# CEA-LIST/runia_core

Measured on AMD Instinct MI355X. Metric: OOD scores/sec, LaREM 16-MC PCA-256 (ResNet-18 layer4 latent 512x4x4), higher is better.
Workload: dtype f64

## Files before the change

### include/runia_hip.h

```cpp
#ifndef RUNIA_HIP_H
#define RUNIA_HIP_H

#include <stddef.h>
#include <stdint.h>

#ifdef __cplusplus
extern "C" {
#endif

#define RUNIA_OK 0
#define RUNIA_E_INVALID (-1)
#define RUNIA_E_LAUNCH (-2)
#define RUNIA_E_NODEVICE (-3)
#define RUNIA_E_WORKSPACE (-4)

typedef void* runia_stream_t;

int runia_abi_version(void);
const char* runia_error_string(int code);
int runia_device_count(void);
int runia_clock_probe(uint64_t* out4, int chain, runia_stream_t stream);
int runia_time_next_launch(void* start_event, void* stop_event);

int runia_mc_stack_f32(const float* x, const float* rand, int64_t rand_image_stride, float* out,
// ... 81 lines not shown
size_t runia_knn_prepared_workspace_bytes(int64_t N, int64_t M, int64_t D, int k);
int runia_knn_kth_prepared_f32(const float* q, const float* bank, const void* state, size_t state_bytes, float* score,
                               void* workspace, size_t workspace_bytes, int64_t N, int64_t M, int64_t D, int k,
                               runia_stream_t stream);
int runia_knn_kth_f32(const float* q, const float* bank, float* score, void* workspace,
                      size_t workspace_bytes, int64_t N, int64_t M, int64_t D, int k,
                      runia_stream_t stream);

int runia_kde_score_f64(const double* train, const double* x, double* score, int64_t M, int64_t N,
                        int64_t D, double bandwidth, runia_stream_t stream);
int runia_kde_score_kernel_f64(const double* train, const double* x, double* score, int64_t M, int64_t N, int64_t D,
                               double bandwidth, int kind, runia_stream_t stream);
int runia_row_sqnorm_f64(const double* x, double* out, int64_t N, int64_t D, runia_stream_t stream);
size_t runia_kde_workspace_bytes(int64_t N, int64_t M);
int runia_kde_score_packed_f64(const double* packed_train_t, const double* train_sqnorm, const double* x,
                               double* score, void* workspace, size_t workspace_bytes, int64_t M, int64_t N,
                               int64_t D, double bandwidth, runia_stream_t stream);

int runia_mc_entropy_supported(int H, int W, int n_mc, int k);
size_t runia_mc_entropy_workspace_bytes(int64_t N, int H, int W, int n_mc);
int runia_mc_mask_table_f32(const float* rand, int64_t rand_image_stride, void* workspace,
                            size_t workspace_bytes, int64_t N, int H, int W, int n_mc, double drop_prob,
                            int block_size, runia_stream_t stream);
int runia_mc_stack_table_f32(const float* x, const float* rand, int64_t rand_image_stride, float* z,
                             void* workspace, size_t workspace_bytes, int64_t N, int C, int H, int W, int n_mc,
                             double drop_prob, int block_size, runia_stream_t stream);
int runia_mc_entropy_from_table_f32(const float* x, const void* workspace, size_t workspace_bytes, double* h,
                                    float* z_out, double* zero_fill, int64_t N, int C, int H, int W, int n_mc,
                                    int k, double min_dist, runia_stream_t stream);
int runia_mc_entropy_f32(const float* x, const float* rand, int64_t rand_image_stride, double* h,
                         float* z_out, double* zero_fill, void* workspace, size_t workspace_bytes, int64_t N,
                         int C, int H, int W, int n_mc, double drop_prob, int block_size, int k, double min_dist,
                         runia_stream_t stream);
int runia_mc_draws_f32(float* out, int64_t N, int n_mc, int H, int W, uint64_t seed, int64_t first_image,
                       runia_stream_t stream);
int runia_mc_mask_table_counter_f32(uint64_t seed, int64_t first_image, void* workspace, size_t workspace_bytes,
                                    int64_t N, int H, int W, int n_mc, double drop_prob, int block_size,
                                    int redraw_dead_layers, runia_stream_t stream);
int runia_mc_entropy_counter_f32(const float* x, uint64_t seed, int64_t first_image, double* h, float* z_out,
                                 double* zero_fill, void* workspace, size_t workspace_bytes, int64_t N, int C, int H,
                                 int W, int n_mc, double drop_prob, int block_size, int k, double min_dist,
                                 int redraw_dead_layers, runia_stream_t stream);
int runia_pca_md_score_f64(const double* h, const double* packed_ct, const double* bias,
                           const double* scale, const double* md_mean, const double* packed_p,
                           double* score, double* y_out, int64_t N, int64_t D, int64_t n,
                           runia_stream_t stream);
size_t runia_proj_sq_workspace_bytes(int64_t N);
int runia_proj_sq_accumulate_f64(const double* h, const double* packed_m, const double* c, double* score,
                                 int64_t N, int64_t D, int64_t r, runia_stream_t stream);
int runia_proj_sq_score_f64(const double* h, const double* packed_m, const double* c, double* score,
                            void* workspace, size_t workspace_bytes, int64_t N, int64_t D, int64_t r,
                            runia_stream_t stream);

size_t runia_covariance_workspace_bytes(int64_t N, int64_t D);
int runia_covariance_f64(const double* x, double* mean, double* cov, void* workspace,
                         size_t workspace_bytes, int64_t N, int64_t D, runia_stream_t stream);
int runia_covariance_f32in(const float* x, double* mean, double* cov, void* workspace,
                           size_t workspace_bytes, int64_t N, int64_t D, runia_stream_t stream);

int runia_roi_align_f32(const float* input, const float* boxes, const int* batch_idx, float* out, int64_t K, int64_t B,
                        int C, int H, int W, int PH, int PW, double spatial_scale, int sampling_ratio, int aligned,
                        runia_stream_t stream);
int runia_nchw_to_nhwc_f32(const float* in, float* out, int64_t B, int C, int64_t HW, runia_stream_t stream);
int runia_roi_mc_entropy_supported(int PH, int PW, int n_mc, int k, int sampling_ratio);
size_t runia_roi_mc_entropy_workspace_bytes(int64_t K, int PH, int PW, int n_mc, int sampling_ratio);
int runia_roi_mc_entropy_f32(const float* feat_nhwc, const float* boxes, const int* batch_idx, const float* rand,
// ... 176 lines not shown
```

### runia_core_amd/_hip.py

```python
from __future__ import annotations

import contextlib
import ctypes
import os
import threading
from ctypes import c_char_p, c_double, c_float, c_int, c_int64, c_size_t, c_uint64, c_void_p
from typing import NamedTuple, Optional, Union

import numpy as np
import torch

from . import config as _config

_LIB_PATH = os.path.join(os.path.dirname(os.path.abspath(__file__)), "librunia_hip.so")
_lib: Optional[ctypes.CDLL] = None

_SIGNATURES = {
    "runia_abi_version": (c_int, []),
    "runia_error_string": (c_char_p, [c_int]),
    "runia_device_count": (c_int, []),
    "runia_clock_probe": (c_int, [c_void_p, c_int, c_void_p]),
    "runia_time_next_launch": (c_int, [c_void_p, c_void_p]),
    "runia_mc_stack_f32": (
        c_int,
# ... 56 lines not shown
    "runia_knn_kth_prepared_f32": (c_int, [c_void_p, c_void_p, c_void_p, c_size_t, c_void_p, c_void_p, c_size_t, c_int64, c_int64,
                                           c_int64, c_int, c_void_p]),
    "runia_knn_kth_f32": (
        c_int,
        [c_void_p, c_void_p, c_void_p, c_void_p, c_size_t, c_int64, c_int64, c_int64, c_int, c_void_p],
    ),
    "runia_kde_score_f64": (c_int, [c_void_p, c_void_p, c_void_p, c_int64, c_int64, c_int64, c_double, c_void_p]),
    "runia_row_sqnorm_f64": (c_int, [c_void_p, c_void_p, c_int64, c_int64, c_void_p]),
    "runia_kde_workspace_bytes": (c_size_t, [c_int64, c_int64]),
    "runia_kde_score_packed_f64": (
        c_int,
        [c_void_p, c_void_p, c_void_p, c_void_p, c_void_p, c_size_t, c_int64, c_int64, c_int64, c_double, c_void_p],
    ),
    "runia_mc_entropy_supported": (c_int, [c_int, c_int, c_int, c_int]),
    "runia_mc_entropy_workspace_bytes": (c_size_t, [c_int64, c_int, c_int, c_int]),
    "runia_mc_mask_table_f32": (
        c_int,
        [c_void_p, c_int64, c_void_p, c_size_t, c_int64, c_int, c_int, c_int, c_double, c_int, c_void_p],
    ),
    "runia_mc_stack_table_f32": (
        c_int,
        [c_void_p, c_void_p, c_int64, c_void_p, c_void_p, c_size_t, c_int64, c_int, c_int, c_int, c_int, c_double, c_int,
         c_void_p],
    ),
    "runia_mc_entropy_from_table_f32": (
        c_int,
        [c_void_p, c_void_p, c_size_t, c_void_p, c_void_p, c_void_p, c_int64, c_int, c_int, c_int, c_int, c_int,
         c_double, c_void_p],
    ),
    "runia_mc_entropy_f32": (
        c_int,
        [c_void_p, c_void_p, c_int64, c_void_p, c_void_p, c_void_p, c_void_p, c_size_t, c_int64, c_int, c_int, c_int,
         c_int, c_double, c_int, c_int, c_double, c_void_p],
    ),
    "runia_mc_draws_f32": (c_int, [c_void_p, c_int64, c_int, c_int, c_int, c_uint64, c_int64, c_void_p]),
    "runia_mc_mask_table_counter_f32": (
        c_int,
        [c_uint64, c_int64, c_void_p, c_size_t, c_int64, c_int, c_int, c_int, c_double, c_int, c_int, c_void_p],
    ),
    "runia_mc_entropy_counter_f32": (
        c_int,
        [c_void_p, c_uint64, c_int64, c_void_p, c_void_p, c_void_p, c_void_p, c_size_t, c_int64, c_int, c_int, c_int,
         c_int, c_double, c_int, c_int, c_double, c_int, c_void_p],
    ),
    "runia_select_hist_f32": (c_int, [c_void_p, c_void_p, c_int64, ctypes.c_uint32, ctypes.c_uint32, c_int, c_void_p]),
    "runia_cholesky_f32": (c_int, [c_void_p, c_void_p, c_int64, c_int64, c_double, c_void_p]),
    "runia_cholesky_f64": (c_int, [c_void_p, c_void_p, c_int64, c_int64, c_double, c_void_p]),
    "runia_gmm_log_prob_workspace_bytes": (c_size_t, [c_int64, c_int64, c_int]),
    "runia_gmm_log_prob_f32": (c_int, [c_void_p, c_void_p, c_void_p, c_void_p, c_void_p, c_void_p, c_void_p, c_size_t, c_int64,
                                       c_int64, c_int, c_void_p]),
    "runia_ood_metrics_workspace_bytes": (c_size_t, [c_int64]),
    "runia_ood_metrics_f64": (c_int, [c_void_p, c_int64, c_void_p, c_int64, c_void_p, c_void_p, c_size_t, c_void_p]),
    "runia_ood_metrics_f32": (c_int, [c_void_p, c_int64, c_void_p, c_int64, c_void_p, c_void_p, c_size_t, c_void_p]),
    "runia_ood_clf_curve_f64": (
        c_int, [c_void_p, c_int64, c_void_p, c_int64, c_void_p, c_void_p, c_void_p, c_void_p, c_void_p, c_size_t, c_void_p]),
    "runia_ood_clf_curve_f32": (
        c_int, [c_void_p, c_int64, c_void_p, c_int64, c_void_p, c_void_p, c_void_p, c_void_p, c_void_p, c_size_t, c_void_p]),
    "runia_eigh_workspace_bytes": (c_size_t, [c_int64]),
    "runia_eigh_init_f64": (c_int, [c_void_p, c_void_p, c_int64, c_void_p, c_size_t, c_void_p]),
    "runia_eigh_sweep_f64": (c_int, [c_void_p, c_void_p, c_int64, c_void_p, c_size_t, c_void_p, c_void_p]),
    "runia_eigh_block_padded": (c_int64, [c_int64]),
    "runia_eigh_block_workspace_bytes": (c_size_t, [c_int64]),
    "runia_eigh_block_init_f64": (c_int, [c_void_p, c_void_p, c_int64, c_void_p, c_size_t, c_void_p]),
    "runia_eigh_block_sweep_f64": (c_int, [c_void_p, c_void_p, c_int64, c_void_p, c_size_t, c_void_p, c_void_p]),
    "runia_matmul_f64": (c_int, [c_void_p, c_void_p, c_void_p, c_int64, c_int64, c_int64, c_int, c_void_p]),
    "runia_p2p_buffer_bytes": (c_size_t, [c_int, c_size_t]),
# ... 803 lines not shown
               min_dist: float = 1e-5, want_samples: bool = False, out: Optional[torch.Tensor] = None,
               kernel_events: Optional[list] = None, zero_fill: Optional[torch.Tensor] = None,
               table: Optional[torch.Tensor] = None):
    lib = load_library()
    require_gpu()
    assert x.is_cuda and x.dtype == torch.float32 and x.dim() == 4
    x = x.contiguous()
    n, c, hh, ww = x.shape
    if table is not None:
        h = torch.empty((n, c), dtype=torch.float64, device=x.device) if out is None else out
        assert h.is_cuda and h.dtype == torch.float64 and h.shape == (n, c) and h.is_contiguous()
        z = torch.empty((n * n_mc, c), dtype=torch.float32, device=x.device) if want_samples else None
        ws_bytes = int(lib.runia_mc_entropy_workspace_bytes(n, hh, ww, n_mc))
        assert table.is_cuda and table.numel() >= ws_bytes and n <= 65535
        if zero_fill is not None:
            assert zero_fill.is_cuda and zero_fill.dtype == torch.float64 and zero_fill.shape == (n,) and zero_fill.is_contiguous()
        args = (x.data_ptr(), table.data_ptr(), ws_bytes, h.data_ptr(), _ptr(z), _ptr(zero_fill), n, c, hh, ww, n_mc, int(k),
                float(min_dist))
        if kernel_events is not None:
            kernel_events.append(_timed_call("runia_mc_entropy_from_table_f32", *args))
        else:
            launch("runia_mc_entropy_from_table_f32", *args)
        return (h, z) if want_samples else h
    counter = rand if isinstance(rand, CounterDraws) else None
    rand, stride = _draws(None if counter is not None else rand, n, n_mc, hh, ww)
    if out is None:
        h = torch.empty((n, c), dtype=torch.float64, device=x.device)
    else:
        assert out.is_cuda and out.dtype == torch.float64 and out.shape == (n, c) and out.is_contiguous()
        h = out
    z = torch.empty((n * n_mc, c), dtype=torch.float32, device=x.device) if want_samples else None
    if zero_fill is not None:
        assert zero_fill.is_cuda and zero_fill.dtype == torch.float64 and zero_fill.shape == (n,) and zero_fill.is_contiguous()
    ws_bytes = int(lib.runia_mc_entropy_workspace_bytes(min(65535, n), hh, ww, n_mc))
    ws = torch.empty(max(ws_bytes, 16), dtype=torch.uint8, device=x.device)
    if counter is not None:
        seed, redraw = int(counter.seed) & (2**64 - 1), int(bool(counter.redraw_dead_layers))
    for done, m in _image_slices(n):
        xp, hp = x.data_ptr() + done * c * hh * ww * 4, h.data_ptr() + done * c * 8
        rp = None if rand is None else rand.data_ptr() + done * stride * 4
        zp = None if z is None else z.data_ptr() + done * n_mc * c * 4
        zf = None if zero_fill is None else zero_fill.data_ptr() + done * 8
        if kernel_events is not None:
            if counter is not None:
                launch("runia_mc_mask_table_counter_f32", seed, int(counter.first_image) + done, ws.data_ptr(), ws_bytes, m, hh,
                       ww, n_mc, float(drop_prob), int(block_size), redraw)
            else:
                launch("runia_mc_mask_table_f32", rp, stride, ws.data_ptr(), ws_bytes, m, hh, ww, n_mc, float(drop_prob),
                       int(block_size))
            kernel_events.append(_timed_call("runia_mc_entropy_from_table_f32", xp, ws.data_ptr(), ws_bytes, hp, zp, zf, m, c, hh,
                                             ww, n_mc, int(k), float(min_dist)))
        elif counter is not None:
            launch("runia_mc_entropy_counter_f32", xp, seed, int(counter.first_image) + done, hp, zp, zf, ws.data_ptr(), ws_bytes,
                   m, c, hh, ww, n_mc, float(drop_prob), int(block_size), int(k), float(min_dist), redraw)
        else:
            launch("runia_mc_entropy_f32", xp, rp, stride, hp, zp, zf, ws.data_ptr(), ws_bytes, m, c, hh, ww, n_mc,
                   float(drop_prob), int(block_size), int(k), float(min_dist))
    return (h, z) if want_samples else h


@_device_guard()
def proj_sq_accumulate(h: torch.Tensor, packed_m: torch.Tensor, c: torch.Tensor, r: int, out: torch.Tensor) -> torch.Tensor:
    require_gpu()
    assert h.is_cuda and h.dtype == torch.float64 and h.dim() == 2
    h = h.contiguous()
    nrow, d = h.shape
    assert out.is_cuda and out.dtype == torch.float64 and out.shape == (nrow,) and out.is_contiguous()
    launch("runia_proj_sq_accumulate_f64", h.data_ptr(), packed_m.data_ptr(), c.data_ptr(), out.data_ptr(), nrow, d, int(r))
    return out


@_device_guard()
def pca_md_score(h: torch.Tensor, packed_ct: Optional[torch.Tensor], bias: Optional[torch.Tensor],
                 scale: Optional[torch.Tensor], md_mean: torch.Tensor, packed_p: torch.Tensor, n: int,
                 want_projection: bool = False, out: Optional[torch.Tensor] = None):
    require_gpu()
    assert h.is_cuda and h.dtype == torch.float64 and h.dim() == 2
    h = h.contiguous()
    nrow, d = h.shape
    if out is None:
        s = torch.empty((nrow,), dtype=torch.float64, device=h.device)
    else:
        assert out.is_cuda and out.dtype == torch.float64 and out.shape == (nrow,) and out.is_contiguous()
        s = out
    y = torch.empty((nrow, n), dtype=torch.float64, device=h.device) if want_projection else None
    launch("runia_pca_md_score_f64", h.data_ptr(), _ptr(packed_ct), _ptr(bias), _ptr(scale), md_mean.data_ptr(),
           packed_p.data_ptr(), s.data_ptr(), _ptr(y), nrow, d, n)
    return (s, y) if want_projection else s


# ... 635 lines not shown
```

### runia_core_amd/csrc/fused.hip

```cpp
#include "common.hpp"
#include "entropy_core.hpp"
#include "mfma_f64_tile.hpp"
#include "philox.hpp"
#include "div_consts.hpp"

namespace {

using namespace runia_entropy;
using namespace runia_mfma;

constexpr int kMaxMC = 64;
typedef float f2 __attribute__((ext_vector_type(2)));

__device__ __forceinline__ void layer_consts(int cnt, int& m, float& flag, float& zh, float& zl) {
  const int a = cnt ? __ffs(cnt) - 1 : 0;
  m = cnt >> a;
  flag = __uint_as_float((unsigned)(127 - a) << 23);
  zh = cnt ? __uint_as_float(runia_div::kDivHi[(m - 1) >> 1]) : NAN;
  zl = cnt ? __uint_as_float(runia_div::kDivLo[(m - 1) >> 1]) : 0.f;
}

__device__ __forceinline__ float add_f32(float a, float b) {
  float r;
  asm("v_add_f32 %0, %1, %2" : "=v"(r) : "v"(a), "v"(b));
// ... 7 lines not shown
}

template <int HT, int WT>
__host__ __device__ constexpr int mask_slot(int p) {
  if constexpr (HT % 2 == 0) {
    const int y = p / WT, xw = p - y * WT;
    return ((y >> 1) * WT + xw) * 2 + (y & 1);
  } else {
    return p;
  }
}

template <int HT, int WT>
__host__ __device__ constexpr int slot_position(int slot) {
  if constexpr (HT % 2 == 0) {
    const int e = slot & 1, t = slot >> 1;
    const int k = t / WT, xw = t - k * WT;
    return (2 * k + e) * WT + xw;
  } else {
    return slot;
  }
}

template <int HT, int WT>
__device__ __forceinline__ unsigned long long columns_below(int k) {
  unsigned long long row = (k >= 64) ? ~0ull : ((1ull << k) - 1ull), m = 0ull;
#pragma unroll
  for (int y = 0; y < HT; ++y) m |= row << (y * WT);
  return m;
}

constexpr int kMaskBitsWaves = 4;

template <int HT, int WT, int NP, bool REDRAW = false>
__global__ __launch_bounds__(64 * kMaskBitsWaves) void mc_mask_bits_kernel(const float* __restrict__ rnd,
                                                                           int64_t rand_stride,
                                                                           float* __restrict__ table, int64_t N,
                                                                           int n_mc, float gamma, int block_size,
                                                                           int identity, int sort_layers,
                                                                           uint64_t rng_seed, int64_t first_image) {
  constexpr int HW = HT * WT;
  static_assert(HW <= 64 && NP <= 64, "one drop layer per 64-bit word");
  constexpr bool DIV = (64 % HW == 0);
  constexpr int WORDS = (NP * HW + 63) / 64;
  constexpr unsigned long long FULL = (HW == 64) ? ~0ull : ((1ull << HW) - 1ull);
  const int lane = threadIdx.x & 63;
  const int64_t img = (int64_t)blockIdx.x * kMaskBitsWaves + (threadIdx.x >> 6);
  if (img >= N) return;
  const int bit0 = lane * HW, word0 = bit0 >> 6, off = bit0 & 63;
  const int pad = block_size / 2;

  auto seeds_of = [&](unsigned attempt) -> unsigned long long {
    float d[WORDS];
    if (rnd) {
      const float* r = rnd + img * rand_stride;
#pragma unroll
      for (int t = 0; t < WORDS; ++t) {
        const int i = lane + 64 * t;
        d[t] = (i < n_mc * HW) ? r[i] : 1.0f;
      }
    } else {
#pragma unroll
      for (int q = 0; q < (WORDS + 3) / 4; ++q) {
        const runia_philox::u4 b = runia_philox::lane_block(rng_seed, (uint64_t)(first_image + img), lane, q, attempt);
#pragma unroll
        for (int j = 0; j < 4; ++j) {
          const int t = 4 * q + j;
          if (t < WORDS) d[t] = (lane + 64 * t < n_mc * HW) ? runia_philox::component(b, j) : 1.0f;
        }
      }
    }
    unsigned long long lo = 0ull, hi = 0ull;
#pragma unroll
    for (int t = 0; t < WORDS; ++t) {
      const unsigned long long w = __ballot(d[t] < gamma);
      if (t == word0) lo = w;
      if (!DIV && t == word0 + 1) hi = w;
    }
    unsigned long long sd = lo >> off;
    if (!DIV && off + HW > 64) sd |= hi << (64 - off);
    return sd & FULL;
// ... 6 lines not shown
      hx |= (ox >= 0) ? ((seed >> ox) & columns_below<HT, WT>(WT - ox))
                      : ((seed << -ox) & ~columns_below<HT, WT>(-ox) & FULL);
    }
    unsigned long long dropped = 0ull;
    for (int dy = 0; dy < block_size; ++dy) {
      const int oy = dy - pad;
      if (oy >= HT || -oy >= HT) continue;
      dropped |= (oy >= 0) ? (hx >> (oy * WT)) : ((hx << (-oy * WT)) & FULL);
    }
    return ~dropped & FULL;
  };

  unsigned long long keep = identity ? FULL : keep_of(seeds_of(0u));
  if (REDRAW && !identity && !rnd) {
    for (unsigned attempt = 1; attempt <= 16u; ++attempt) {
      if (__ballot(lane < n_mc && keep == 0ull) == 0ull) break;
      const unsigned long long again = keep_of(seeds_of(attempt));
      if (keep == 0ull) keep = again;
    }
  }
  const int cnt = __popcll(keep);
  int m;
  float flag, zh, zl;
  layer_consts(cnt, m, flag, zh, zl);
  const int key = m ? m : 127;
  int rank = 0;
#pragma unroll
  for (int j = 0; j < NP; ++j) {
    const int o = __shfl(key, j, 64);
    rank += (j < n_mc) && ((o < key) || (o == key && j < lane));
  }
  if (!sort_layers) rank = lane;
  if (lane >= n_mc) return;
  float* out = table + img * (int64_t)(n_mc * (HW + 2));
  float* rec = out + rank * HW;
  if constexpr (HW % 4 == 0) {
#pragma unroll
    for (int c = 0; c < HW / 4; ++c) {
      float4 v;
      v.x = ((keep >> slot_position<HT, WT>(4 * c)) & 1ull) ? flag : 0.f;
      v.y = ((keep >> slot_position<HT, WT>(4 * c + 1)) & 1ull) ? flag : 0.f;
      v.z = ((keep >> slot_position<HT, WT>(4 * c + 2)) & 1ull) ? flag : 0.f;
      v.w = ((keep >> slot_position<HT, WT>(4 * c + 3)) & 1ull) ? flag : 0.f;
      reinterpret_cast<float4*>(rec)[c] = v;
    }
  } else {
#pragma unroll
    for (int q = 0; q < HW; ++q) rec[q] = ((keep >> slot_position<HT, WT>(q)) & 1ull) ? flag : 0.f;
  }
  out[n_mc * HW + rank] = zh;
  out[n_mc * (HW + 1) + rank] = zl;
}

#ifndef K1_BLOCK
#define K1_BLOCK 128
#endif
constexpr int kK1Block = K1_BLOCK;

struct RoiSource {
  const float* nhwc;
  const unsigned* table;
  int64_t image_bytes;
  int C;
  int roi_dwords;
};

template <int HT, int WT, int G>
__device__ __forceinline__ void roi_load_map(float (&u)[HT * WT], const RoiSource* __restrict__ src, int64_t roi, int c) {
  typedef const __attribute__((address_space(4))) unsigned* cptr;
  cptr tab = (cptr)(src->table + roi * (int64_t)src->roi_dwords);
  const unsigned image = tab[0];
  const __amdgpu_buffer_rsrc_t rsrc = __builtin_amdgcn_make_buffer_rsrc(
      const_cast<float*>(src->nhwc) + (int64_t)image * (src->image_bytes / 4), 0, (int)src->image_bytes, 0x00020000);
  const int voff = c * 4;
  cptr rows = tab + 8, cols = tab + 8 + 4 * (HT * G);
  constexpr float count = (float)(G * G);
  constexpr int SX = WT * G, SY = HT * G;
  unsigned ox_lo[SX], ox_hi[SX];
  float hx[SX], lx[SX];
#pragma unroll
  for (int sx = 0; sx < SX; ++sx) {
    ox_lo[sx] = cols[4 * sx];
    ox_hi[sx] = cols[4 * sx + 1];
    hx[sx] = __uint_as_float(cols[4 * sx + 2]);
// ... 14 lines not shown
        for (int sx = 0; sx < SX; ++sx) { tl[sx][0] = th[sx][0]; tl[sx][1] = th[sx][1]; }
      } else {
#pragma unroll
        for (int sx = 0; sx < SX; ++sx) {
          tl[sx][0] = __builtin_bit_cast(float, __builtin_amdgcn_raw_buffer_load_b32(rsrc, voff, (int)(oy_lo + ox_lo[sx]), 0));
          tl[sx][1] = __builtin_bit_cast(float, __builtin_amdgcn_raw_buffer_load_b32(rsrc, voff, (int)(oy_lo + ox_hi[sx]), 0));
        }
      }
#pragma unroll
      for (int sx = 0; sx < SX; ++sx) {
        th[sx][0] = __builtin_bit_cast(float, __builtin_amdgcn_raw_buffer_load_b32(rsrc, voff, (int)(oy_hi + ox_lo[sx]), 0));
        th[sx][1] = __builtin_bit_cast(float, __builtin_amdgcn_raw_buffer_load_b32(rsrc, voff, (int)(oy_hi + ox_hi[sx]), 0));
      }
      cur_lo = oy_lo;
      cur_hi = oy_hi;
    }
    __builtin_amdgcn_sched_barrier(0);
#pragma unroll
    for (int sx = 0; sx < SX; ++sx) {
      const float w1 = hy * hx[sx], w2 = hy * lx[sx], w3 = ly * hx[sx], w4 = ly * lx[sx];
      const float val = w1 * tl[sx][0] + w2 * tl[sx][1] + w3 * th[sx][0] + w4 * th[sx][1];
      float& bin = acc[(sy / G) * WT + (sx / G)];
      bin += val;
      asm volatile("" : "+v"(bin));
    }
  }
#pragma unroll
  for (int p = 0; p < HT * WT; ++p) u[p] = acc[p] / count;
}

#ifndef K1_IMGS
#define K1_IMGS 1
#endif
template <int HT, int WT, int NP, int K, bool FULL, bool ENTROPY, int ROI_G>
__device__ __forceinline__ void mc_entropy_item(const float* __restrict__ x, const float* __restrict__ table,
                                                double* __restrict__ h, float* __restrict__ z_out,
                                                double* __restrict__ zero_fill, int64_t N, int C, int n_mc_rt,
                                                double min_dist, double const_term, double inv_n, int64_t img, int c) {
  constexpr int HW = HT * WT;
  constexpr bool PAIRS = (HT % 2 == 0);
  const int n_mc = FULL ? NP : n_mc_rt;
  if (img >= N) return;
  if (zero_fill && c == 0) zero_fill[img] = 0.0;
  if (c >= C) return;
  const float* mk = table + img * (int64_t)(n_mc * (HW + 2));
  const float* zhs = mk + n_mc * HW;
  const float* zls = zhs + n_mc;
  float u[HW];
  if constexpr (ROI_G > 0) {
    roi_load_map<HT, WT, ROI_G>(u, reinterpret_cast<const RoiSource*>(x), img, c);
  } else {
    const float* xc = x + (img * C + c) * (int64_t)HW;
    if constexpr (HW % 4 == 0) {
#pragma unroll
      for (int p = 0; p < HW / 4; ++p) {
        const float4 v = reinterpret_cast<const float4*>(xc)[p];
        u[4 * p] = v.x; u[4 * p + 1] = v.y; u[4 * p + 2] = v.z; u[4 * p + 3] = v.w;
      }
    } else {
#pragma unroll
      for (int p = 0; p < HW; ++p) u[p] = xc[p];
    }
  }
  constexpr bool w_pow2 = (WT & (WT - 1)) == 0, h_pow2 = (HT & (HT - 1)) == 0;
  constexpr bool hw_pow2 = w_pow2 && h_pow2;
  if constexpr (!hw_pow2) {
#pragma unroll
    for (int p = 0; p < HW; ++p) u[p] *= (float)HW;
  }
  const float rW = 1.0f / (float)WT, rH = 1.0f / (float)HT;
  float z[NP];
  float q[PAIRS ? 1 : HW];
  f2 q2[PAIRS ? HW / 2 : 1];
  unsigned cur_zh_bits = __float_as_uint(1.0f);
#pragma unroll
  for (int p = 0; p < HW; ++p) {
    if constexpr (PAIRS) q2[mask_slot<HT, WT>(p) >> 1][mask_slot<HT, WT>(p) & 1] = u[p];
    else q[p] = u[p];
  }
#ifndef K1_GCAP
#define K1_GCAP 128
#endif
  constexpr int GCAP = FULL ? K1_GCAP : K1_GCAP / 2;
  constexpr int G = (GCAP / HW < 1) ? 1 : ((GCAP / HW > NP) ? NP : GCAP / HW);
  if constexpr (!(FULL && NP % G == 0)) {
#pragma unroll
    for (int s = 0; s < NP; ++s) z[s] = INFINITY;
  }
#ifndef K1_TRIP_UNROLL
#define K1_TRIP_UNROLL 1
#endif
#pragma unroll K1_TRIP_UNROLL
  for (int s0 = 0; s0 < NP; s0 += G) {
    float znew[G];
    float dg[G], rg[G], mg[G][HW];
    const float* mk_t = mk + (FULL ? s0 * HW : 0);
    const float* zhs_t = zhs + (FULL ? s0 : 0);
    const float* zls_t = zls + (FULL ? s0 : 0);
#pragma unroll
    for (int g = 0; g < G; ++g) {
      const int sc = FULL ? g : ((s0 + g < n_mc) ? s0 + g : n_mc - 1);
      dg[g] = zhs_t[sc];
      rg[g] = zls_t[sc];
#pragma unroll
      for (int p = 0; p < HW; ++p) mg[g][p] = mk_t[sc * HW + p];
    }
#pragma unroll
    for (int g = 0; g < G; ++g) {
      const int s = s0 + g;
      znew[g] = INFINITY;
      if (FULL || s < n_mc) {
        const float zh = dg[g], zl = rg[g];
        if (__float_as_uint(zh) != cur_zh_bits) {
#pragma unroll
          for (int p = 0; p < HW; ++p) {
            const float qv = fmaf(u[p], zh, u[p] * zl);
            if constexpr (PAIRS) q2[mask_slot<HT, WT>(p) >> 1][mask_slot<HT, WT>(p) & 1] = qv;
            else q[p] = qv;
          }
          cur_zh_bits = __float_as_uint(zh);
        }
        const float* m = mg[g];
        float col;
        if constexpr (PAIRS) {
          float rows[HT];
#pragma unroll
          for (int k2 = 0; k2 < HT / 2; ++k2) {
            const f2* qq = q2 + k2 * WT;
            const float* mm = m + 2 * k2 * WT;
            f2 acc = qq[0] * (f2){mm[0], mm[1]};
#pragma unroll
// ... 38 lines not shown
#pragma unroll
    for (int i = NP - 1; i >= G; --i) z[i] = z[i - G];
#pragma unroll
    for (int g = 0; g < G; ++g) z[g] = znew[g];
  }
  if constexpr (ENTROPY) {
    float nan_probe = z[0];
#pragma unroll
    for (int s = 1; s < NP; ++s) nan_probe += z[s];
    const bool bad = nan_probe != nan_probe;
    sort_asc<NP>(z);
    double res = const_term + inv_n * column_log_sum<NP, K, FULL>(z, n_mc, min_dist);
    if (bad) res = NAN;
    h[img * C + c] = res;
  }
}

template <int HT, int WT, int NP, int K, bool FULL, bool ENTROPY = true, int ROI_G = 0>
#ifdef K1_WAVES
__attribute__((amdgpu_waves_per_eu(K1_WAVES, 8)))
#endif
__global__ __launch_bounds__(kK1Block) void mc_entropy_kernel(const float* __restrict__ x,
                                                          const float* __restrict__ table,
                                                          double* __restrict__ h, float* __restrict__ z_out,
                                                          double* __restrict__ zero_fill, int64_t N, int C,
                                                          int n_mc_rt, double min_dist, double const_term,
                                                          double inv_n) {
  const unsigned chunks = (unsigned)(C + kK1Block - 1) / kK1Block;
  const unsigned slot = blockIdx.x >> 3;
  const int c = (int)(slot % chunks) * kK1Block + threadIdx.x;
#pragma unroll 1
  for (int rep = 0; rep < K1_IMGS; ++rep) {
    const int64_t img = ((int64_t)(slot / chunks) * K1_IMGS + rep) * 8 + (blockIdx.x & 7);
    mc_entropy_item<HT, WT, NP, K, FULL, ENTROPY, ROI_G>(x, table, h, z_out, zero_fill, N, C, n_mc_rt, min_dist, const_term,
                                                        inv_n, img, c);
  }
}

struct PcaMdArgs {
  const double* h;
  const double* packed_ct;
  const double* bias;
  const double* scale;
  const double* md_mean;
  const double* packed_p;
  double* score;
  double* y_out;
  int64_t N, D, n;
};

template <int RT>
__global__ __launch_bounds__(256) void pca_md_kernel(PcaMdArgs g) {
  constexpr int BM = 16 * RT;
  extern __shared__ double lds[];
  const int64_t n_pad = n_padded(g.n);
  const int ypitch = (int)n_pad + 2;
  double* lds_a = lds;
  double* lds_y = lds + 2 * BM * APITCH;
  double* part = lds_y + (size_t)BM * ypitch;
  const int tid = threadIdx.x, lane = tid & 63;
  const int wave = __builtin_amdgcn_readfirstlane(tid >> 6);
  const int li = lane & 15, lg = lane >> 4;
  const int64_t NT = n_pad / 16;
  const int64_t r0 = (int64_t)blockIdx.x * BM;

  if (g.packed_ct) {
    const int64_t nchunks = k_padded(g.D) / KC;
    constexpr int PER_T = BM * KC / 256;
    for (int64_t cb = 0; cb < n_pad / BN; ++cb) {
// ... 431 lines not shown
#undef RUNIA_MCE
  return RUNIA_E_INVALID;
}

extern "C" int runia_mc_entropy_from_table_f32(const float* x, const void* workspace, size_t workspace_bytes,
                                               double* h, float* z_out, double* zero_fill, int64_t N, int C,
                                               int H, int W, int n_mc, int k, double min_dist,
                                               runia_stream_t stream) {
  if (C <= 0 || k < 1 || k >= n_mc) return RUNIA_E_INVALID;
  if (int rc = mc_args_ok(N, H, W, n_mc, workspace, workspace_bytes)) return rc;
  if (N == 0) return RUNIA_OK;
  if (!x || !h) return RUNIA_E_INVALID;
  if (!runia_mc_entropy_supported(H, W, n_mc, k)) return RUNIA_E_INVALID;
  const float* table = reinterpret_cast<const float*>(workspace);
  const double ct = digamma_diff(n_mc, k), inv_n = 1.0 / (double)n_mc;
  const unsigned grid = (unsigned)((((N + 7) / 8 + K1_IMGS - 1) / K1_IMGS) * 8 * ((C + kK1Block - 1) / kK1Block));
  hipStream_t s = as_stream(stream);
  const bool x16 = ((((uintptr_t)x) & 15) == 0);
#define RUNIA_MCE(HH, WW, NPP, KK)                                                                          \
  if (H == HH && W == WW && n_mc <= NPP && n_mc > NPP / 2 && k == KK && (x16 || (HH * WW) % 4 != 0)) {      \
    if (n_mc == NPP)                                                                                        \
      RUNIA_LAUNCH_TIMED((mc_entropy_kernel<HH, WW, NPP, KK, true>), grid, kK1Block, 0, s, x, table, h, z_out, \
                         zero_fill, N, C, n_mc, min_dist, ct, inv_n);                                       \
    else                                                                                                    \
      RUNIA_LAUNCH_TIMED((mc_entropy_kernel<HH, WW, NPP, KK, false>), grid, kK1Block, 0, s, x, table, h, z_out, \
                         zero_fill, N, C, n_mc, min_dist, ct, inv_n);                                       \
    return runia_check_launch();                                                                            \
  }
  RUNIA_MCE_SHAPES(RUNIA_MCE)
#undef RUNIA_MCE
  return RUNIA_E_INVALID;
}

extern "C" int runia_mc_entropy_f32(const float* x, const float* rnd, int64_t rand_image_stride, double* h,
                                    float* z_out, double* zero_fill, void* workspace, size_t workspace_bytes,
                                    int64_t N, int C, int H, int W, int n_mc, double drop_prob, int block_size,
                                    int k, double min_dist, runia_stream_t stream) {
  if (N < 0 || C <= 0 || H <= 0 || W <= 0 || n_mc < 2 || n_mc > kMaxMC || block_size < 1 || k < 1 || k >= n_mc)
    return RUNIA_E_INVALID;
  if (N == 0) return RUNIA_OK;
  if (!x || !h || N > 65535) return RUNIA_E_INVALID;
  if (!runia_mc_entropy_supported(H, W, n_mc, k)) return RUNIA_E_INVALID;
  if (drop_prob != 0.0 && !rnd) return RUNIA_E_INVALID;
  if (!(((((uintptr_t)x) & 15) == 0) || (H * W) % 4 != 0)) return RUNIA_E_INVALID;
  if (int rc = runia_mc_mask_table_f32(rnd, rand_image_stride, workspace, workspace_bytes, N, H, W, n_mc, drop_prob,
                                       block_size, stream))
    return rc;
  return runia_mc_entropy_from_table_f32(x, workspace, workspace_bytes, h, z_out, zero_fill, N, C, H, W, n_mc, k,
                                         min_dist, stream);
}

int runia_roi_sample_table(const float* feat_nhwc, const float* boxes, const int* batch_idx, void* table, size_t table_bytes,
                           int64_t K, int64_t B, int C, int H, int W, int PH, int PW, double spatial_scale, int G, int aligned,
                           hipStream_t s);
size_t runia_roi_sample_table_bytes(int64_t K, int PH, int PW, int G);

#define RUNIA_ROI_MCE_SHAPES(X)                                                                                    \
  X(7, 7, 16, 5, 2) X(7, 7, 32, 5, 2) X(7, 7, 16, 5, 1) X(7, 7, 32, 5, 1)                                          \
  X(4, 4, 16, 5, 2) X(4, 4, 32, 5, 2) X(8, 8, 16, 5, 2) X(8, 8, 32, 5, 2)

extern "C" int runia_roi_mc_entropy_supported(int PH, int PW, int n_mc, int k, int sampling_ratio) {
  if (!runia_mc_entropy_supported(PH, PW, n_mc, k)) return 0;
#define RUNIA_ROI_HAS(HH, WW, NPP, KK, GG) \
  if (PH == HH && PW == WW && n_mc <= NPP && n_mc > NPP / 2 && k == KK && sampling_ratio == GG) return 1;
  RUNIA_ROI_MCE_SHAPES(RUNIA_ROI_HAS)
#undef RUNIA_ROI_HAS
  return 0;
}
extern "C" size_t runia_roi_mc_entropy_workspace_bytes(int64_t K, int PH, int PW, int n_mc, int sampling_ratio) {
  if (K <= 0 || sampling_ratio < 1) return 0;
  const size_t masks = (runia_mc_entropy_workspace_bytes(K, PH, PW, n_mc) + 255) / 256 * 256;
  return masks + runia_roi_sample_table_bytes(K, PH, PW, sampling_ratio);
}
extern "C" int runia_roi_mc_entropy_f32(const float* feat_nhwc, const float* boxes, const int* batch_idx, const float* rnd,
                                        int64_t rand_image_stride, double* h, float* z_out, void* workspace,
                                        size_t workspace_bytes, int64_t K, int64_t B, int C, int H, int W, int PH, int PW,
                                        double spatial_scale, int sampling_ratio, int aligned, int n_mc, double drop_prob,
                                        int block_size, int k, double min_dist, runia_stream_t stream) {
  if (K < 0 || B <= 0 || C <= 0 || H <= 0 || W <= 0 || n_mc < 2 || n_mc > kMaxMC || block_size < 1 || k < 1 || k >= n_mc)
    return RUNIA_E_INVALID;
  if (K == 0) return RUNIA_OK;
  if (!feat_nhwc || !boxes || !h || K > 65535 || (B > 1 && !batch_idx)) return RUNIA_E_INVALID;
// ... 34 lines not shown
                                  runia_stream_t stream) {
  if (N < 0 || n_mc < 1 || H <= 0 || W <= 0 || first_image < 0 || (int64_t)n_mc * H * W > (1 << 20))
    return RUNIA_E_INVALID;
  if (N == 0) return RUNIA_OK;
  if (!out) return RUNIA_E_INVALID;
  const int64_t total = N * n_mc * H * W;
  if ((total + 255) / 256 > 0x7fffffffLL) return RUNIA_E_INVALID;
  mc_draws_kernel<<<(unsigned)((total + 255) / 256), 256, 0, as_stream(stream)>>>(out, N, n_mc * H * W, seed,
                                                                                first_image);
  return runia_check_launch();
}

extern "C" int runia_mc_mask_table_counter_f32(uint64_t seed, int64_t first_image, void* workspace,
                                               size_t workspace_bytes, int64_t N, int H, int W, int n_mc,
                                               double drop_prob, int block_size, int redraw_dead_layers,
                                               runia_stream_t stream) {
  if (first_image < 0) return RUNIA_E_INVALID;
  return mc_mask_table(nullptr, 0, workspace, workspace_bytes, N, H, W, n_mc, drop_prob, block_size, 1, stream, true,
                       seed, first_image, redraw_dead_layers ? 1 : 0);
}

extern "C" int runia_mc_entropy_counter_f32(const float* x, uint64_t seed, int64_t first_image, double* h,
                                            float* z_out, double* zero_fill, void* workspace, size_t workspace_bytes,
                                            int64_t N, int C, int H, int W, int n_mc, double drop_prob,
                                            int block_size, int k, double min_dist, int redraw_dead_layers,
                                            runia_stream_t stream) {
  if (N < 0 || C <= 0 || H <= 0 || W <= 0 || n_mc < 2 || n_mc > kMaxMC || block_size < 1 || k < 1 || k >= n_mc ||
      first_image < 0)
    return RUNIA_E_INVALID;
  if (N == 0) return RUNIA_OK;
  if (!x || !h || N > 65535) return RUNIA_E_INVALID;
  if (!runia_mc_entropy_supported(H, W, n_mc, k)) return RUNIA_E_INVALID;
  if (!(((((uintptr_t)x) & 15) == 0) || (H * W) % 4 != 0)) return RUNIA_E_INVALID;
  if (int rc = runia_mc_mask_table_counter_f32(seed, first_image, workspace, workspace_bytes, N, H, W, n_mc,
                                               drop_prob, block_size, redraw_dead_layers, stream))
    return rc;
  return runia_mc_entropy_from_table_f32(x, workspace, workspace_bytes, h, z_out, zero_fill, N, C, H, W, n_mc, k,
                                         min_dist, stream);
}

extern "C" int runia_mc_entropy_supported(int H, int W, int n_mc, int k) {
  if (k != 5 || k >= n_mc) return 0;
  const bool hw = (H == 4 && W == 4);
  if (hw && n_mc > 4 && n_mc <= 32) return 1;
  if (n_mc > 8 && n_mc <= 32 && ((H == 2 && W == 2) || (H == 7 && W == 7) || (H == 8 && W == 8))) return 1;
  return 0;
}

static bool proj_sq_dma_ok(int64_t D, int64_t r) {
  return K2_DMA && D % KC == 0 && D < (1 << 23) && packed_elems(D, r) < ((int64_t)1 << 29);
}
static bool proj_sq_one_round(unsigned grid) { return (int64_t)grid <= (int64_t)K2_WAVES_DMA * runia_cu_count(); }
template <int RT, int NCT, bool ACCUMULATE, bool SPLIT>
static void launch_proj_sq(unsigned grid, hipStream_t s, const ProjSqArgs& g, bool dma) {
  if (dma && (RT > 1 || proj_sq_one_round(grid))) proj_sq_kernel<RT, NCT, ACCUMULATE, SPLIT, true><<<grid, 256, 0, s>>>(g);
  else proj_sq_kernel<RT, NCT, ACCUMULATE, SPLIT, false><<<grid, 256, 0, s>>>(g);
}

static bool proj_sq_large_tiles(int64_t N, int64_t cus) {
  const int64_t tiles32 = (N + 31) / 32;
  const int64_t rounds = (tiles32 + cus - 1) / cus;
  return tiles32 >= 2 * cus && 100 * tiles32 >= 93 * rounds * cus;
}

extern "C" int runia_proj_sq_accumulate_f64(const double* h, const double* packed_m, const double* c, double* score,
                                            int64_t N, int64_t D, int64_t r, runia_stream_t stream) {
// ... 42 lines not shown
```

Before: 57.93 million.

## Fuse mask-table build into MC entropy kernel with producer blocks and ready tags

Replaces the two-kernel sequence (mask-table build, then entropy from table) with one kernel. Leading producer blocks build and publish each image's mask record with agent-scope stores and a per-image ready tag. Consumer blocks check the tag and rebuild the record themselves if it is not yet ready, then read the record through a constant address-space pointer. This removes one launch and the inter-kernel dependency, at the cost of redundant mask work when consumers race ahead, extra workspace for tags, and a fallback when the stream is being captured.

```diff
diff --git a/include/runia_hip.h b/include/runia_hip.h
--- a/include/runia_hip.h
+++ b/include/runia_hip.h
@@ -137,6 +137,11 @@
                          float* z_out, double* zero_fill, void* workspace, size_t workspace_bytes, int64_t N,
                          int C, int H, int W, int n_mc, double drop_prob, int block_size, int k, double min_dist,
                          runia_stream_t stream);
+size_t runia_mc_entropy_inline_workspace_bytes(int64_t N, int H, int W, int n_mc);
+int runia_mc_entropy_f32_mode(const float* x, const float* rand, int64_t rand_image_stride, double* h,
+                              float* z_out, double* zero_fill, void* workspace, size_t workspace_bytes, int64_t N,
+                              int C, int H, int W, int n_mc, double drop_prob, int block_size, int k, double min_dist,
+                              int mode, runia_stream_t stream);
 int runia_mc_draws_f32(float* out, int64_t N, int n_mc, int H, int W, uint64_t seed, int64_t first_image,
                        runia_stream_t stream);
 int runia_mc_mask_table_counter_f32(uint64_t seed, int64_t first_image, void* workspace, size_t workspace_bytes,
diff --git a/runia_core_amd/_hip.py b/runia_core_amd/_hip.py
--- a/runia_core_amd/_hip.py
+++ b/runia_core_amd/_hip.py
@@ -112,6 +112,12 @@
         c_int,
         [c_void_p, c_void_p, c_int64, c_void_p, c_void_p, c_void_p, c_void_p, c_size_t, c_int64, c_int, c_int, c_int,
          c_int, c_double, c_int, c_int, c_double, c_void_p],
+    ),
+    "runia_mc_entropy_inline_workspace_bytes": (c_size_t, [c_int64, c_int, c_int, c_int]),
+    "runia_mc_entropy_f32_mode": (
+        c_int,
+        [c_void_p, c_void_p, c_int64, c_void_p, c_void_p, c_void_p, c_void_p, c_size_t, c_int64, c_int, c_int, c_int,
+         c_int, c_double, c_int, c_int, c_double, c_int, c_void_p],
     ),
     "runia_mc_draws_f32": (c_int, [c_void_p, c_int64, c_int, c_int, c_int, c_uint64, c_int64, c_void_p]),
     "runia_mc_mask_table_counter_f32": (
@@ -981,7 +987,7 @@
     z = torch.empty((n * n_mc, c), dtype=torch.float32, device=x.device) if want_samples else None
     if zero_fill is not None:
         assert zero_fill.is_cuda and zero_fill.dtype == torch.float64 and zero_fill.shape == (n,) and zero_fill.is_contiguous()
-    ws_bytes = int(lib.runia_mc_entropy_workspace_bytes(min(65535, n), hh, ww, n_mc))
+    ws_bytes = int(lib.runia_mc_entropy_inline_workspace_bytes(min(65535, n), hh, ww, n_mc))
     ws = torch.empty(max(ws_bytes, 16), dtype=torch.uint8, device=x.device)
     if counter is not None:
         seed, redraw = int(counter.seed) & (2**64 - 1), int(bool(counter.redraw_dead_layers))
@@ -990,21 +996,18 @@
         rp = None if rand is None else rand.data_ptr() + done * stride * 4
         zp = None if z is None else z.data_ptr() + done * n_mc * c * 4
         zf = None if zero_fill is None else zero_fill.data_ptr() + done * 8
+        if counter is not None:
+            name = "runia_mc_entropy_counter_f32"
+            args = (xp, seed, int(counter.first_image) + done, hp, zp, zf, ws.data_ptr(), ws_bytes, m, c, hh, ww, n_mc,
+                    float(drop_prob), int(block_size), int(k), float(min_dist), redraw)
+        else:
+            name = "runia_mc_entropy_f32"
+            args = (xp, rp, stride, hp, zp, zf, ws.data_ptr(), ws_bytes, m, c, hh, ww, n_mc, float(drop_prob),
+                    int(block_size), int(k), float(min_dist))
         if kernel_events is not None:
-            if counter is not None:
-                launch("runia_mc_mask_table_counter_f32", seed, int(counter.first_image) + done, ws.data_ptr(), ws_bytes, m, hh,
-                       ww, n_mc, float(drop_prob), int(block_size), redraw)
-            else:
-                launch("runia_mc_mask_table_f32", rp, stride, ws.data_ptr(), ws_bytes, m, hh, ww, n_mc, float(drop_prob),
-                       int(block_size))
-            kernel_events.append(_timed_call("runia_mc_entropy_from_table_f32", xp, ws.data_ptr(), ws_bytes, hp, zp, zf, m, c, hh,
-                                             ww, n_mc, int(k), float(min_dist)))
-        elif counter is not None:
-            launch("runia_mc_entropy_counter_f32", xp, seed, int(counter.first_image) + done, hp, zp, zf, ws.data_ptr(), ws_bytes,
-                   m, c, hh, ww, n_mc, float(drop_prob), int(block_size), int(k), float(min_dist), redraw)
+            kernel_events.append(_timed_call(name, *args))
         else:
-            launch("runia_mc_entropy_f32", xp, rp, stride, hp, zp, zf, ws.data_ptr(), ws_bytes, m, c, hh, ww, n_mc,
-                   float(drop_prob), int(block_size), int(k), float(min_dist))
+            launch(name, *args)
     return (h, z) if want_samples else h
 
 
diff --git a/runia_core_amd/csrc/fused.hip b/runia_core_amd/csrc/fused.hip
--- a/runia_core_amd/csrc/fused.hip
+++ b/runia_core_amd/csrc/fused.hip
@@ -63,21 +63,25 @@
 
 constexpr int kMaskBitsWaves = 4;
 
-template <int HT, int WT, int NP, bool REDRAW = false>
-__global__ __launch_bounds__(64 * kMaskBitsWaves) void mc_mask_bits_kernel(const float* __restrict__ rnd,
-                                                                           int64_t rand_stride,
-                                                                           float* __restrict__ table, int64_t N,
-                                                                           int n_mc, float gamma, int block_size,
-                                                                           int identity, int sort_layers,
-                                                                           uint64_t rng_seed, int64_t first_image) {
+template <typename T>
+__device__ __forceinline__ void store_agent(T* p, T v) {
+  __hip_atomic_store(p, v, __ATOMIC_RELAXED, __HIP_MEMORY_SCOPE_AGENT);
+}
+__device__ __forceinline__ unsigned long long pack2(float lo, float hi) {
+  return (unsigned long long)__float_as_uint(lo) | ((unsigned long long)__float_as_uint(hi) << 32);
+}
+
+template <int HT, int WT, int NP, bool REDRAW, bool PUBLISH = false>
+__device__ __forceinline__ void build_mask_record(const float* __restrict__ rnd, int64_t rand_stride,
+                                                  float* __restrict__ out, int64_t img, int n_mc, float gamma,
+                                                  int block_size, int identity, int sort_layers, uint64_t rng_seed,
+                                                  int64_t first_image) {
   constexpr int HW = HT * WT;
   static_assert(HW <= 64 && NP <= 64, "one drop layer per 64-bit word");
   constexpr bool DIV = (64 % HW == 0);
   constexpr int WORDS = (NP * HW + 63) / 64;
   constexpr unsigned long long FULL = (HW == 64) ? ~0ull : ((1ull << HW) - 1ull);
   const int lane = threadIdx.x & 63;
-  const int64_t img = (int64_t)blockIdx.x * kMaskBitsWaves + (threadIdx.x >> 6);
-  if (img >= N) return;
   const int bit0 = lane * HW, word0 = bit0 >> 6, off = bit0 & 63;
   const int pad = block_size / 2;
 
@@ -150,7 +154,6 @@
   }
   if (!sort_layers) rank = lane;
   if (lane >= n_mc) return;
-  float* out = table + img * (int64_t)(n_mc * (HW + 2));
   float* rec = out + rank * HW;
   if constexpr (HW % 4 == 0) {
 #pragma unroll
@@ -160,14 +163,41 @@
       v.y = ((keep >> slot_position<HT, WT>(4 * c + 1)) & 1ull) ? flag : 0.f;
       v.z = ((keep >> slot_position<HT, WT>(4 * c + 2)) & 1ull) ? flag : 0.f;
       v.w = ((keep >> slot_position<HT, WT>(4 * c + 3)) & 1ull) ? flag : 0.f;
-      reinterpret_cast<float4*>(rec)[c] = v;
+      if constexpr (PUBLISH) {
+        store_agent(reinterpret_cast<unsigned long long*>(rec) + 2 * c, pack2(v.x, v.y));
+        store_agent(reinterpret_cast<unsigned long long*>(rec) + 2 * c + 1, pack2(v.z, v.w));
+      } else {
+        reinterpret_cast<float4*>(rec)[c] = v;
+      }
     }
   } else {
 #pragma unroll
-    for (int q = 0; q < HW; ++q) rec[q] = ((keep >> slot_position<HT, WT>(q)) & 1ull) ? flag : 0.f;
-  }
-  out[n_mc * HW + rank] = zh;
-  out[n_mc * (HW + 1) + rank] = zl;
+    for (int q = 0; q < HW; ++q) {
+      const float v = ((keep >> slot_position<HT, WT>(q)) & 1ull) ? flag : 0.f;
+      if constexpr (PUBLISH) store_agent(rec + q, v);
+      else rec[q] = v;
+    }
+  }
+  if constexpr (PUBLISH) {
+    store_agent(out + n_mc * HW + rank, zh);
+    store_agent(out + n_mc * (HW + 1) + rank, zl);
+  } else {
+    out[n_mc * HW + rank] = zh;
+    out[n_mc * (HW + 1) + rank] = zl;
+  }
+}
+
+template <int HT, int WT, int NP, bool REDRAW = false>
+__global__ __launch_bounds__(64 * kMaskBitsWaves) void mc_mask_bits_kernel(const float* __restrict__ rnd,
+                                                                           int64_t rand_stride,
+                                                                           float* __restrict__ table, int64_t N,
+                                                                           int n_mc, float gamma, int block_size,
+                                                                           int identity, int sort_layers,
+                                                                           uint64_t rng_seed, int64_t first_image) {
+  const int64_t img = (int64_t)blockIdx.x * kMaskBitsWaves + (threadIdx.x >> 6);
+  if (img >= N) return;
+  build_mask_record<HT, WT, NP, REDRAW>(rnd, rand_stride, table + img * (int64_t)(n_mc * (HT * WT + 2)), img, n_mc, gamma,
+                                        block_size, identity, sort_layers, rng_seed, first_image);
 }
 
 #ifndef K1_BLOCK
@@ -248,8 +278,8 @@
 #ifndef K1_IMGS
 #define K1_IMGS 1
 #endif
-template <int HT, int WT, int NP, int K, bool FULL, bool ENTROPY, int ROI_G>
-__device__ __forceinline__ void mc_entropy_item(const float* __restrict__ x, const float* __restrict__ table,
+template <int HT, int WT, int NP, int K, bool FULL, bool ENTROPY, int ROI_G, typename REC>
+__device__ __forceinline__ void mc_entropy_item(const float* __restrict__ x, REC rec,
                                                 double* __restrict__ h, float* __restrict__ z_out,
                                                 double* __restrict__ zero_fill, int64_t N, int C, int n_mc_rt,
                                                 double min_dist, double const_term, double inv_n, int64_t img, int c) {
@@ -259,9 +289,9 @@
   if (img >= N) return;
   if (zero_fill && c == 0) zero_fill[img] = 0.0;
   if (c >= C) return;
-  const float* mk = table + img * (int64_t)(n_mc * (HW + 2));
-  const float* zhs = mk + n_mc * HW;
-  const float* zls = zhs + n_mc;
+  const REC mk = rec;
+  const REC zhs = mk + n_mc * HW;
+  const REC zls = zhs + n_mc;
   float u[HW];
   if constexpr (ROI_G > 0) {
     roi_load_map<HT, WT, ROI_G>(u, reinterpret_cast<const RoiSource*>(x), img, c);
@@ -310,9 +340,9 @@
   for (int s0 = 0; s0 < NP; s0 += G) {
     float znew[G];
     float dg[G], rg[G], mg[G][HW];
-    const float* mk_t = mk + (FULL ? s0 * HW : 0);
-    const float* zhs_t = zhs + (FULL ? s0 : 0);
-    const float* zls_t = zls + (FULL ? s0 : 0);
+    const REC mk_t = mk + (FULL ? s0 * HW : 0);
+    const REC zhs_t = zhs + (FULL ? s0 : 0);
+    const REC zls_t = zls + (FULL ? s0 : 0);
 #pragma unroll
     for (int g = 0; g < G; ++g) {
       const int sc = FULL ? g : ((s0 + g < n_mc) ? s0 + g : n_mc - 1);
@@ -417,9 +447,71 @@
 #pragma unroll 1
   for (int rep = 0; rep < K1_IMGS; ++rep) {
     const int64_t img = ((int64_t)(slot / chunks) * K1_IMGS + rep) * 8 + (blockIdx.x & 7);
-    mc_entropy_item<HT, WT, NP, K, FULL, ENTROPY, ROI_G>(x, table, h, z_out, zero_fill, N, C, n_mc_rt, min_dist, const_term,
+    const float* rec = table + img * (int64_t)((FULL ? NP : n_mc_rt) * (HT * WT + 2));
+    mc_entropy_item<HT, WT, NP, K, FULL, ENTROPY, ROI_G>(x, rec, h, z_out, zero_fill, N, C, n_mc_rt, min_dist, const_term,
                                                         inv_n, img, c);
   }
+}
+
+struct MaskDraws {
+  const float* rnd;
+  int64_t rand_stride;
+  uint64_t rng_seed;
+  int64_t first_image;
+  float gamma;
+  int block_size;
+  int identity;
+};
+
+constexpr int kInlineWaves = kK1Block / 64;
+
+__device__ __forceinline__ void publish_record(unsigned long long* word, unsigned long long tag) {
+  __builtin_amdgcn_fence(__ATOMIC_RELEASE, "workgroup");
+  asm volatile("s_waitcnt vmcnt(0)" ::: "memory");
+  if ((threadIdx.x & 63) == 0) store_agent(word, tag);
+}
+
+template <int HT, int WT, int NP, int K, bool FULL, bool REDRAW>
+__attribute__((amdgpu_waves_per_eu((HT * WT <= 16 && NP <= 16) ? 6 : 1, 8)))
+__global__ __launch_bounds__(kK1Block) void mc_entropy_inline_kernel(const float* __restrict__ x, float* table,
+                                                                   unsigned long long* ready, unsigned long long tag0,
+                                                                   unsigned producers, int read_ready, MaskDraws d,
+                                                                   double* __restrict__ h, float* __restrict__ z_out,
+                                                                   double* __restrict__ zero_fill, int64_t N, int C,
+                                                                   int n_mc_rt, double min_dist, double const_term,
+                                                                   double inv_n) {
+  constexpr int HW = HT * WT;
+  const int n_mc = FULL ? NP : n_mc_rt;
+  const int64_t rec_floats = n_mc * (HW + 2);
+  if (blockIdx.x < producers) {
+    const int64_t img = (int64_t)blockIdx.x * kInlineWaves + (threadIdx.x >> 6);
+    if (img >= N) return;
+    build_mask_record<HT, WT, NP, REDRAW, true>(d.rnd, d.rand_stride, table + img * rec_floats, img, n_mc, d.gamma,
+                                                d.block_size, d.identity, 1, d.rng_seed, d.first_image);
+    publish_record(ready + img, tag0 + (unsigned long long)img);
+    return;
+  }
+  const unsigned bid = blockIdx.x - producers;
+  const unsigned chunks = (unsigned)(C + kK1Block - 1) / kK1Block;
+  const unsigned slot = bid >> 3;
+  const int c = (int)(slot % chunks) * kK1Block + threadIdx.x;
+  const int64_t img = (int64_t)(slot / chunks) * 8 + (bid & 7);
+  if (img >= N) return;
+  float* rec = table + img * rec_floats;
+  const unsigned long long tag = tag0 + (unsigned long long)img;
+  unsigned long long seen = ~tag;
+  if (read_ready) seen = __hip_atomic_load(ready + img, __ATOMIC_RELAXED, __HIP_MEMORY_SCOPE_AGENT);
+  if (__ballot(seen != tag) != 0ull) {
+    build_mask_record<HT, WT, NP, REDRAW, true>(d.rnd, d.rand_stride, rec, img, n_mc, d.gamma, d.block_size, d.identity, 1,
+                                                d.rng_seed, d.first_image);
+    publish_record(ready + img, tag);
+  }
+  __builtin_amdgcn_fence(__ATOMIC_ACQUIRE, "workgroup");
+  uintptr_t addr = reinterpret_cast<uintptr_t>(rec);
+  asm volatile("" : "+s"(addr)::"memory");
+  typedef const __attribute__((address_space(4))) float* const_rec;
+  mc_entropy_item<HT, WT, NP, K, FULL, true, 0>(x, (const_rec)addr, h, z_out, zero_fill, N, C, n_mc_rt, min_dist, const_term,
+                                                inv_n, img, c);
 }
 
 struct PcaMdArgs {
@@ -917,10 +1009,85 @@
   return RUNIA_E_INVALID;
 }
 
-extern "C" int runia_mc_entropy_f32(const float* x, const float* rnd, int64_t rand_image_stride, double* h,
-                                    float* z_out, double* zero_fill, void* workspace, size_t workspace_bytes,
-                                    int64_t N, int C, int H, int W, int n_mc, double drop_prob, int block_size,
-                                    int k, double min_dist, runia_stream_t stream) {
+extern "C" size_t runia_mc_entropy_inline_workspace_bytes(int64_t N, int H, int W, int n_mc) {
+  const size_t table = runia_mc_entropy_workspace_bytes(N, H, W, n_mc);
+  if (table == 0) return 0;
+  return (table + 63) / 64 * 64 + (size_t)N * sizeof(unsigned long long);
+}
+
+static unsigned long long mc_inline_tag() {
+  static std::atomic<unsigned long long> launches{0};
+  unsigned long long z = launches.fetch_add(1, std::memory_order_relaxed) + 1;
+  z = (z ^ (z >> 30)) * 0xbf58476d1ce4e5b9ull;
+  z = (z ^ (z >> 27)) * 0x94d049bb133111ebull;
+  return z ^ (z >> 31);
+}
+
+static bool mc_inline_ok(const void* workspace, size_t workspace_bytes, int64_t N, int H, int W, int n_mc, hipStream_t s) {
+  if (!workspace || (((uintptr_t)workspace) & 63) != 0) return false;
+  if (((size_t)n_mc * (size_t)(H * W + 2) * sizeof(float)) % 64 != 0) return false;
+  if (workspace_bytes < runia_mc_entropy_inline_workspace_bytes(N, H, W, n_mc)) return false;
+  hipStreamCaptureStatus cap = hipStreamCaptureStatusNone;
+  if (hipStreamIsCapturing(s, &cap) != hipSuccess) {
+    (void)hipGetLastError();
+    return false;
+  }
+  return cap == hipStreamCaptureStatusNone;
+}
+
+enum { kInlineAuto = 0, kInlineSelfBuild = 1, kInlineAllReady = 2 };
+
+static int mc_entropy_inline(const float* x, const float* rnd, int64_t rand_image_stride, bool counter, uint64_t seed,
+                             int64_t first_image, int redraw, double* h, float* z_out, double* zero_fill, void* workspace,
+                             int64_t N, int C, int H, int W, int n_mc, double drop_prob, int block_size, int k,
+                             double min_dist, int mode, hipStream_t s) {
+  MaskDraws d;
+  d.identity = (drop_prob == 0.0);
+  if (!d.identity && !rnd && !counter) return RUNIA_E_INVALID;
+  d.rnd = counter ? nullptr : rnd;
+  d.rand_stride = rand_image_stride;
+  d.rng_seed = seed;
+  d.first_image = first_image;
+  d.gamma = (float)(drop_prob / (double)(block_size * block_size));
+  d.block_size = block_size;
+  float* table = reinterpret_cast<float*>(workspace);
+  const size_t table_bytes = runia_mc_entropy_workspace_bytes(N, H, W, n_mc);
+  unsigned long long* ready =
+      reinterpret_cast<unsigned long long*>(reinterpret_cast<char*>(workspace) + (table_bytes + 63) / 64 * 64);
+  const unsigned long long tag0 = mc_inline_tag();
+  const double ct = digamma_diff(n_mc, k), inv_n = 1.0 / (double)n_mc;
+  const unsigned consumers = (unsigned)(((N + 7) / 8) * 8 * ((C + kK1Block - 1) / kK1Block));
+  const unsigned producers = (unsigned)(((N + kInlineWaves - 1) / kInlineWaves + 7) / 8 * 8);
+  const bool redraw_k = counter && redraw && !d.identity;
+#define RUNIA_MCE_INLINE(HH, WW, NPP, KK, FULL_, REDRAW_)                                                            \
+  do {                                                                                                               \
+    auto kern = mc_entropy_inline_kernel<HH, WW, NPP, KK, FULL_, REDRAW_>;                                            \
+    if (mode == kInlineAllReady)                                                                                     \
+      hipLaunchKernelGGL(kern, dim3(producers), dim3(kK1Block), 0, s, x, table, ready, tag0, producers, 1, d, h,     \
+                         z_out, zero_fill, N, C, n_mc, min_dist, ct, inv_n);                                         \
+    const unsigned prod = (mode == kInlineAuto) ? producers : 0u;                                                    \
+    RUNIA_LAUNCH_TIMED(kern, prod + consumers, kK1Block, 0, s, x, table, ready, tag0, prod,                          \
+                       (mode == kInlineSelfBuild) ? 0 : 1, d, h, z_out, zero_fill, N, C, n_mc, min_dist, ct, inv_n); \
+  } while (0)
+#define RUNIA_MCE(HH, WW, NPP, KK)                                                                          \
+  if (H == HH && W == WW && n_mc <= NPP && n_mc > NPP / 2 && k == KK) {                                     \
+    if (n_mc == NPP) {                                                                                      \
+      if (redraw_k) RUNIA_MCE_INLINE(HH, WW, NPP, KK, true, true);                                          \
+      else RUNIA_MCE_INLINE(HH, WW, NPP, KK, true, false);                                                  \
+    } else {                                                                                                \
+      if (redraw_k) RUNIA_MCE_INLINE(HH, WW, NPP, KK, false, true);                                         \
+      else RUNIA_MCE_INLINE(HH, WW, NPP, KK, false, false);                                                 \
+    }                                                                                                       \
+    return runia_check_launch();                                                                            \
+  }
+  RUNIA_MCE_SHAPES(RUNIA_MCE)
+#undef RUNIA_MCE
+#undef RUNIA_MCE_INLINE
+  return RUNIA_E_INVALID;
+}
+
+static int mc_entropy_f32_checks(const float* x, const float* rnd, const double* h, int64_t N, int C, int H, int W,
+                                 int n_mc, double drop_prob, int block_size, int k) {
   if (N < 0 || C <= 0 || H <= 0 || W <= 0 || n_mc < 2 || n_mc > kMaxMC || block_size < 1 || k < 1 || k >= n_mc)
     return RUNIA_E_INVALID;
   if (N == 0) return RUNIA_OK;
@@ -928,11 +1095,35 @@
   if (!runia_mc_entropy_supported(H, W, n_mc, k)) return RUNIA_E_INVALID;
   if (drop_prob != 0.0 && !rnd) return RUNIA_E_INVALID;
   if (!(((((uintptr_t)x) & 15) == 0) || (H * W) % 4 != 0)) return RUNIA_E_INVALID;
+  return RUNIA_OK;
+}
+
+extern "C" int runia_mc_entropy_f32(const float* x, const float* rnd, int64_t rand_image_stride, double* h,
+                                    float* z_out, double* zero_fill, void* workspace, size_t workspace_bytes,
+                                    int64_t N, int C, int H, int W, int n_mc, double drop_prob, int block_size,
+                                    int k, double min_dist, runia_stream_t stream) {
+  if (int rc = mc_entropy_f32_checks(x, rnd, h, N, C, H, W, n_mc, drop_prob, block_size, k)) return rc;
+  if (N == 0) return RUNIA_OK;
+  if (mc_inline_ok(workspace, workspace_bytes, N, H, W, n_mc, as_stream(stream)))
+    return mc_entropy_inline(x, rnd, rand_image_stride, false, 0, 0, 0, h, z_out, zero_fill, workspace, N, C, H, W, n_mc,
+                             drop_prob, block_size, k, min_dist, kInlineAuto, as_stream(stream));
   if (int rc = runia_mc_mask_table_f32(rnd, rand_image_stride, workspace, workspace_bytes, N, H, W, n_mc, drop_prob,
                                        block_size, stream))
     return rc;
   return runia_mc_entropy_from_table_f32(x, workspace, workspace_bytes, h, z_out, zero_fill, N, C, H, W, n_mc, k,
                                          min_dist, stream);
+}
+
+extern "C" int runia_mc_entropy_f32_mode(const float* x, const float* rnd, int64_t rand_image_stride, double* h,
+                                         float* z_out, double* zero_fill, void* workspace, size_t workspace_bytes,
+                                         int64_t N, int C, int H, int W, int n_mc, double drop_prob, int block_size,
+                                         int k, double min_dist, int mode, runia_stream_t stream) {
+  if (mode != kInlineAuto && mode != kInlineSelfBuild && mode != kInlineAllReady) return RUNIA_E_INVALID;
+  if (int rc = mc_entropy_f32_checks(x, rnd, h, N, C, H, W, n_mc, drop_prob, block_size, k)) return rc;
+  if (N == 0) return RUNIA_OK;
+  if (!mc_inline_ok(workspace, workspace_bytes, N, H, W, n_mc, as_stream(stream))) return RUNIA_E_WORKSPACE;
+  return mc_entropy_inline(x, rnd, rand_image_stride, false, 0, 0, 0, h, z_out, zero_fill, workspace, N, C, H, W, n_mc,
+                           drop_prob, block_size, k, min_dist, mode, as_stream(stream));
 }
 
 int runia_roi_sample_table(const float* feat_nhwc, const float* boxes, const int* batch_idx, void* table, size_t table_bytes,
@@ -1033,6 +1224,10 @@
   if (!x || !h || N > 65535) return RUNIA_E_INVALID;
   if (!runia_mc_entropy_supported(H, W, n_mc, k)) return RUNIA_E_INVALID;
   if (!(((((uintptr_t)x) & 15) == 0) || (H * W) % 4 != 0)) return RUNIA_E_INVALID;
+  if (mc_inline_ok(workspace, workspace_bytes, N, H, W, n_mc, as_stream(stream)))
+    return mc_entropy_inline(x, nullptr, 0, true, seed, first_image, redraw_dead_layers ? 1 : 0, h, z_out, zero_fill,
+                             workspace, N, C, H, W, n_mc, drop_prob, block_size, k, min_dist, kInlineAuto,
+                             as_stream(stream));
   if (int rc = runia_mc_mask_table_counter_f32(seed, first_image, workspace, workspace_bytes, N, H, W, n_mc,
                                                drop_prob, block_size, redraw_dead_layers, stream))
     return rc;
```

New measurement: 55.92 million. 0.965x the previous value.
